# lyf8118/BDS-3-B1C-B2a-SDR-receiver

Hardware: AMD Instinct MI355X
Metric: IF Msamples/s through acquisition (all PRNs x Doppler bins) (higher is better)
Workload: dtype f32

## Files before the change

bds-3-b1c-b2a-sdr-receiver_amd/csrc/bds_acq.hip:

```cpp
#include <hip/hip_runtime.h>

#include <algorithm>
#include <array>
#include <cmath>
#include <cstdarg>
#include <cstdlib>
#include <map>
#include <set>
#include <tuple>

#include "bds_acq_scols.h"
#include "bds_acq_wcols.h"
#include "bds_acq_refine.h"
#include "bds_acq_wrows.h"
#include "bds_acq_pfa.h"
#include "bds_internal.h"

namespace bds {

static const double kPi = 3.14159265358979323846;

#include "bds_acq_plan.h"

struct EventPool {
// ... 1074 lines not shown
        dim3 gr(pl.L1, nb), gc(pl.ntiles, nb);
        if (ncomp == 2) {
            hipLaunchKernelGGL(k_rows_inv<2>, gr, dim3(pl.nt_rows), pl.lds_rows, s_main, pl.p2, pl.twl,
                               (const float2 *)a.d_Xs, pl.L, b0, Cs, a.d_Bw);
            hipLaunchKernelGGL(k_cols_inv_max<2>, gc, dim3(pl.nt_cols), pl.lds_cols, s_main, pl.p1, pl.L2, pl.logT,
                               pl.Spad, (const float2 *)a.d_Bw, pl.L, w0, w1, lo1, hi1, lo2, hi2, recs, pl.ntiles);
        } else {
            hipLaunchKernelGGL(k_rows_inv<1>, gr, dim3(pl.nt_rows), pl.lds_rows, s_main, pl.p2, pl.twl,
                               (const float2 *)a.d_Xs, pl.L, b0, Cs, a.d_Bw);
            hipLaunchKernelGGL(k_cols_inv_max<1>, gc, dim3(pl.nt_cols), pl.lds_cols, s_main, pl.p1, pl.L2, pl.logT,
                               pl.Spad, (const float2 *)a.d_Bw, pl.L, w0, w1, lo1, hi1, lo2, hi2, recs, pl.ntiles);
        }
    }
}

void AcqRun::launch_list(int ncells, Rec *recs, const CellList &cl, int cell0, hipEvent_t mid) {
    Plan2D &pl = a.plan;
    const hipStream_t s_main = stream();
    SieveOut so1 = so;
    so1.recs = recs;
    so1.cell0 = cell0;
    so1.mid = mid;
    if (mid) mids = true;
    const int hi1 = cl.rng ? -1 : (int)a.N - 1, lo2 = cl.rng ? 0 : 1, hi2 = cl.rng ? -1 : 0;
    if (pfa) {
        const int gc = std::max(1, cl.gc), chunks = (ncells + gc - 1) / gc;
        const size_t rows_lds = 2 * 3136 * sizeof(float2);
        want_lds(ctx, pfa::k_pfa_cols<2, false>, pfa::kColsLds);
        pfa::RowsArgs ra{(const uint32_t *)a.d_Xs, (const uint32_t *)a.d_Cs, (uint32_t *)a.d_Bw, cl.bin, cl.cs, ncells, gc, pfa};
        hipLaunchKernelGGL(pfa::k_pfa_rows<2>, dim3((unsigned)(pfa::MP * pfa::K2 * chunks)), dim3(pfa::kRowsThreads), rows_lds, s_main, ra);
        if (mid) (void)hipEventRecord(mid, s_main);
        const int qch = ctx->tune.pfa_qchunk > 0 ? ctx->tune.pfa_qchunk : 1;
        const long items = (long)((pfa::kTiles + qch - 1) / qch) * qch * ncells;
        const unsigned cgrid = (unsigned)std::min<long>(items, ctx->tune.pfa_cgrid > 0 ? ctx->tune.pfa_cgrid : std::max<long>(512, std::min<long>(8192, items / 24)));
        pfa::ColsArgs ca{(const uint32_t *)a.d_Bw, a.d_pfa_coef, ncells, w0, w1, so1.cellmax, so1.lb, so1.lb_div, so1.extra, so1.extra_count,
                         so1.extra_cap, cell0, so1.keep, qch, nullptr, nullptr, -1, -1};
        hipLaunchKernelGGL((pfa::k_pfa_cols<2, false>), dim3(cgrid), dim3(pfa::kColsThreads), pfa::kColsLds, s_main, ca);
        return;
    }
    if (a.half) {
        if (ncomp == 2)
            launch_fast_f<2, __half2>(ctx, s_main, pl, a.d_Xs, ncells, 0, a.d_Cs, a.d_Bw, a.sB, w0, w1, 0, hi1, lo2, hi2, so1, cl);
        else
            launch_fast_f<1, __half2>(ctx, s_main, pl, a.d_Xs, ncells, 0, a.d_Cs, a.d_Bw, a.sB, w0, w1, 0, hi1, lo2, hi2, so1, cl);
    } else {
        if (ncomp == 2)
            launch_fast_f<2, float2>(ctx, s_main, pl, a.d_Xs, ncells, 0, a.d_Cs, a.d_Bw, a.sB, w0, w1, 0, hi1, lo2, hi2, so1, cl);
        else
            launch_fast_f<1, float2>(ctx, s_main, pl, a.d_Xs, ncells, 0, a.d_Cs, a.d_Bw, a.sB, w0, w1, 0, hi1, lo2, hi2, so1, cl);
    }
}

int AcqRun::search() {
    Plan2D &pl = a.plan;
    const hipStream_t s_main = stream();
    int rc;
    const long sample_every = std::max<long>(1, n_pairs_total / kSamples);
    long pair_idx = 0, group_idx = 0;
    if (!multiprn && (rc = ensure_fit(ctx, &a.d_Bw, &a.bw_cap, bw_batches(a, ctx->tune) * (size_t)pl.L))) return rc;
    if (multiprn) {
        for (;;) {
            const size_t need = ((size_t)PB * D * cell_elems * elem + 7) / 8;
            if (!(rc = ensure_fit(ctx, &a.d_Bw, &a.bw_cap, std::max(need, bw_batches(a, ctx->tune) * (size_t)pl.L)))) break;
            if (PB <= 2) return rc;
            (void)hipGetLastError();
            PB = (PB + 1) / 2;
            a.pb_last = PB;
// ... 370 lines not shown
```

bds-3-b1c-b2a-sdr-receiver_amd/csrc/bds_acq_pfa.h:

```cpp
#pragma once

#include <hip/hip_fp16.h>
#include <hip/hip_runtime.h>

#include <type_traits>

#include "bds_acq_wcols.h"

namespace bds {
namespace pfa {

constexpr int K1 = 53, K2 = 12, K3 = 3125;
constexpr long NP = (long)K1 * K2 * K3;
constexpr int MP = 27;
constexpr int NB = 7;
constexpr int kTileLags = 16, kTiles = (K3 + kTileLags - 1) / kTileLags;
constexpr size_t kCellElems = (size_t)kTiles * MP * K2 * kTileLags * 4;
__host__ __device__ constexpr size_t bw_piece(int mp, int k2, int t3) {
    return (((size_t)(t3 / kTileLags) * MP + mp) * K2 + k2) * (kTileLags * 4) + (size_t)(t3 % kTileLags) * 4;
}
constexpr int kRowsThreads = 256, kColsThreads = 256;
constexpr int kCoefFrags = NB * 4 * 2;
constexpr size_t kCoefBytes = (size_t)kCoefFrags * 64 * 16;
constexpr size_t kColsLds = kCoefBytes + (size_t)NB * kColsThreads * 4;

typedef _Float16 h8 __attribute__((ext_vector_type(8)));
typedef float f4 __attribute__((ext_vector_type(4)));

__host__ __device__ inline long lag_of(int t1, int t2, int t3) {
    return ((long)t1 * (NP / K1) + (long)t2 * (NP / K2) + (long)t3 * (NP / K3)) % NP;
}

__device__ __forceinline__ void pk_radix5(v2f &x0, v2f &x1, v2f &x2, v2f &x3, v2f &x4) {
    constexpr float c1 = 0.30901699437494745f, c2 = -0.80901699437494734f, s1 = 0.95105651629515353f, s2 = 0.58778525229247314f;
    const v2f t1 = x1 + x4, t2 = x2 + x3, t3 = x1 - x4, t4 = x2 - x3;
    const v2f m1 = x0 + c1 * t1 + c2 * t2;
    const v2f m2 = x0 + c2 * t1 + c1 * t2;
    const v2f n1 = s1 * t3 + s2 * t4;
    const v2f n2 = s2 * t3 - s1 * t4;
    x0 = x0 + t1 + t2;
    x1 = pk_addj(m1, n1);
    x4 = pk_subj(m1, n1);
    x2 = pk_addj(m2, n2);
    x3 = pk_subj(m2, n2);
}

__device__ __forceinline__ v2f w25(int k) {
    constexpr float c[17] = {1.f, 0.9685831611286311f, 0.8763066800438636f, 0.7289686274214116f, 0.5358267949789965f, 0.30901699437494745f,
                             0.06279051952931353f, -0.1873813145857246f, -0.4257792915650727f, -0.6374239897486897f, -0.8090169943749473f,
                             -0.9297764858882513f, -0.9921147013144778f, -0.9921147013144779f, -0.9297764858882515f, -0.8090169943749478f,
                             -0.6374239897486895f};
    constexpr float s[17] = {0.f, 0.2486898871648548f, 0.4817536741017153f, 0.6845471059286886f, 0.8443279255020151f, 0.9510565162951535f,
                             0.9980267284282716f, 0.9822872507286887f, 0.9048270524660195f, 0.7705132427757893f, 0.5877852522924732f,
                             0.36812455268467814f, 0.12533323356430454f, -0.12533323356430429f, -0.3681245526846779f, -0.5877852522924727f,
                             -0.7705132427757894f};
    return (v2f){c[k], s[k]};
}

__device__ __forceinline__ void pk_radix25(v2f (&x)[25]) {
#pragma unroll
    for (int q0 = 0; q0 < 5; ++q0) pk_radix5(x[q0], x[q0 + 5], x[q0 + 10], x[q0 + 15], x[q0 + 20]);
#pragma unroll
    for (int q0 = 1; q0 < 5; ++q0)
#pragma unroll
// ... 141 lines not shown
#pragma unroll
            for (int sl = 0; sl < 25; ++sl) {
                const int tq = slot25_index(sl);
                typedef _Float16 h2 __attribute__((ext_vector_type(2)));
                outp[c][tq] = __builtin_bit_cast(uint32_t, __builtin_convertvector(x[sl], h2));
            }
        }
        asm volatile("" : "+v"(bin_next));
        bin_cur = __builtin_amdgcn_readfirstlane(bin_next);
        typedef int v4i __attribute__((ext_vector_type(4)));
        const unsigned long long dst_base = (unsigned long long)(A.Bw + (size_t)cell * kCellElems + bw_piece(mp, k2, 0));
        const v4i dst_words = {(int)(unsigned)dst_base, (int)((unsigned)(dst_base >> 32) & 0xffffu), (int)(unsigned)((kCellElems - bw_piece(mp, k2, 0)) * 4), 0x00020000};
#pragma unroll
        for (int e = 0; e < 25; e += 2) {
            uint32_t P[2], Q[2];
#pragma unroll
            for (int c = 0; c < 2; ++c) {
                const uint32_t pe = c < NC ? outp[c < NC ? c : 0][e] : 0u, qo = (c < NC && e + 1 < 25) ? outp[c < NC ? c : 0][e + 1 < 25 ? e + 1 : e] : 0u;
                const auto r = __builtin_amdgcn_permlane32_swap(pe, qo, false, false);
                P[c] = r[0], Q[c] = r[1];
            }
            const int tq = e + half;
            if (live && tq < 25) {
                typedef uint32_t u4 __attribute__((ext_vector_type(4)));
                const int t3s = j + 125 * tq;
                asm volatile("buffer_store_dwordx4 %0, %1, %2, 0 offen\n s_nop 0" ::"v"((u4){P[0], Q[0], P[1], Q[1]}), "v"((int)(bw_piece(0, 0, t3s) * 4)), "s"(dst_words)
                             : "memory");
            }
        }
        __syncthreads();
    }
}

inline void make_coef_frags(uint16_t *out ) {
    auto f2h = [](float f) { return __half_as_ushort(__float2half_rn(f)); };
    auto h2f = [](uint16_t h) { return __half2float(__ushort_as_half(h)); };
    for (int nb = 0; nb < NB; ++nb)
        for (int ins = 0; ins < 4; ++ins)
            for (int lane = 0; lane < 64; ++lane)
                for (int e = 0; e < 8; ++e) {
                    const int kap = 32 * ins + 8 * (lane >> 4) + e, o = 16 * nb + (lane & 15);
                    const int k1 = kap >> 1, ri = kap & 1, t1 = o >> 1, ro = o & 1;
                    double v = 0.0;
                    if (k1 < K1 && t1 < K1) {
                        const double ang = 2.0 * M_PI * (double)((k1 * t1) % K1) / K1;
                        const double c = cos(ang), s = sin(ang);
                        v = ro == 0 ? (ri == 0 ? c : -s) : (ri == 0 ? s : c);
                    }
                    const uint16_t hi = f2h((float)v);
                    const uint16_t lo = f2h((float)(v - (double)h2f(hi)));
                    out[((((size_t)nb * 4 + ins) * 2 + 0) * 64 + lane) * 8 + e] = hi;
                    out[((((size_t)nb * 4 + ins) * 2 + 1) * 64 + lane) * 8 + e] = lo;
                }
}

struct ColsArgs {
    const uint32_t *Bw;
    const uint4 *coef;
    int ncells;
    float w0, w1;
    unsigned long long *cellmax;
    float *lb;
    int lb_div;
    Extra *extra;
    int *extra_count;
    int extra_cap;
    int cell0;
    float keep;
    int qchunk;
    unsigned long long *stats;
    float *dbg;
    int dbg_cell, dbg_group;
};

__device__ __forceinline__ void real_dft6(float a0, float a1, float a2, float a3, float a4, float a5, float (&re)[4], float (&im)[4]) {
    constexpr float h3 = 0.86602540378443865f;
    const float s0 = a0 + a3, d0 = a0 - a3, s1 = a1 + a4, d1 = a1 - a4, s2 = a2 + a5, d2 = a2 - a5;
    const float s12 = s1 + s2, d12 = d1 - d2;
    re[0] = s0 + s12, im[0] = 0.f;
    re[2] = fmaf(-0.5f, s12, s0), im[2] = h3 * (s1 - s2);
    re[1] = fmaf(0.5f, d12, d0), im[1] = h3 * (d1 + d2);
    re[3] = d0 - d12, im[3] = 0.f;
}
__device__ __forceinline__ void real_dft12(const float (&v)[12], float (&P)[7], float (&Q)[7]) {
    float er[4], ei[4], orr[4], oi[4];
    real_dft6(v[0], v[2], v[4], v[6], v[8], v[10], er, ei);
    real_dft6(v[1], v[3], v[5], v[7], v[9], v[11], orr, oi);
    constexpr float c1 = 0.86602540378443865f, s1 = 0.5f;
    P[0] = er[0] + orr[0], Q[0] = 0.f;
    P[6] = er[0] - orr[0], Q[6] = 0.f;
    P[3] = er[3], Q[3] = orr[3];
    P[1] = er[1] + c1 * orr[1] - s1 * oi[1], Q[1] = ei[1] + c1 * oi[1] + s1 * orr[1];
    P[5] = er[1] - c1 * orr[1] + s1 * oi[1], Q[5] = -ei[1] + c1 * oi[1] + s1 * orr[1];
    P[2] = er[2] + s1 * orr[2] - c1 * oi[2], Q[2] = ei[2] + s1 * oi[2] + c1 * orr[2];
    P[4] = er[2] - s1 * orr[2] + c1 * oi[2], Q[4] = -ei[2] + s1 * oi[2] + c1 * orr[2];
}

template <int NC, bool DBG>
__global__ __launch_bounds__(kColsThreads, 2) void k_pfa_cols(ColsArgs A) {
    extern __shared__ __align__(16) unsigned char pfa_lds[];
    uint4 *s_coef = reinterpret_cast<uint4 *>(pfa_lds);
    float *s_bm = reinterpret_cast<float *>(pfa_lds + kCoefBytes);
    const int tid = threadIdx.x, wave = tid >> 6, lane = tid & 63;
    for (int i = tid; i < kCoefFrags * 64; i += kColsThreads) s_coef[i] = A.coef[i];
    __syncthreads();
    const int ai = lane & 15, g = ai >> 2, r = ai & 3, ks = lane >> 4;
    const bool odd = lane & 1;
    auto t2_of = [&](int i) { return odd ? (i == 0 ? 6 : 12 - i) : i; };
    constexpr int kBlocks = kTiles;
    const int qch = A.qchunk > 0 ? A.qchunk : 1, nq = (kBlocks + qch - 1) / qch;
    const unsigned ncl = (unsigned)A.ncells, uq = (unsigned)qch;
    unsigned b = blockIdx.x % uq, cl = (blockIdx.x / uq) % ncl, q = blockIdx.x / (uq * ncl);
    const unsigned gb = gridDim.x % uq, gcl = (gridDim.x / uq) % ncl, gq = gridDim.x / (uq * ncl);
    for (; q < (unsigned)nq; b += gb, cl += gcl + (b >= uq ? (b -= uq, 1u) : 0u), q += gq + (cl >= ncl ? (cl -= ncl, 1u) : 0u)) {
        const int blk = (int)(q * uq + b);
        const int t0 = 16 * blk + 4 * wave;
        if (blk >= kBlocks || t0 >= K3) continue;
        const int cell = A.cell0 + cl;
        float *const lbp = A.lb + cell / A.lb_div;
        const int t3 = min(t0 + g, K3 - 1);
        const uint32_t *base = A.Bw + (size_t)cl * kCellElems;
        uint4 fa[2][3][4];
#pragma unroll
        for (int quad = 0; quad < 3; ++quad)
#pragma unroll
            for (int ins = 0; ins < 4; ++ins) {
                const int mg = 4 * ins + ks;
                const size_t off = bw_piece(0, 4 * quad + r, t3);
                const uint4 l0 = *reinterpret_cast<const uint4 *>(base + (size_t)min(2 * mg, MP - 1) * K2 * (kTileLags * 4) + off);
                const uint4 l1 = *reinterpret_cast<const uint4 *>(base + (size_t)min(2 * mg + 1, MP - 1) * K2 * (kTileLags * 4) + off);
                fa[0][quad][ins] = make_uint4(l0.x, l0.y, l1.x, l1.y);
                fa[1][quad][ins] = make_uint4(l0.z, l0.w, l1.z, l1.w);
            }
        auto matrix = [&](int nb, f4 (&acc2)[NC][3], auto parts_tag) {
            constexpr int PARTS = decltype(parts_tag)::value;
            uint4 fb[4][2];
#pragma unroll
            for (int ins = 0; ins < 4; ++ins)
#pragma unroll
                for (int part = 0; part < PARTS; ++part) fb[ins][part] = s_coef[((nb * 4 + ins) * 2 + part) * 64 + lane];
#pragma unroll
            for (int c = 0; c < NC; ++c) {
#pragma unroll
                for (int quad = 0; quad < 3; ++quad) acc2[c][quad] = (f4){0.f, 0.f, 0.f, 0.f};
#pragma unroll
                for (int ins = 0; ins < 4; ++ins)
#pragma unroll
                    for (int part = 0; part < PARTS; ++part)
#pragma unroll
                        for (int quad = 0; quad < 3; ++quad)
                            acc2[c][quad] = __builtin_amdgcn_mfma_f32_16x16x32_f16(__builtin_bit_cast(h8, fa[c][quad][ins]), __builtin_bit_cast(h8, fb[ins][part]),
                                                                                   acc2[c][quad], 0, 0, 0);
            }
        };
        auto epilogue = [&](const f4 (&acc2)[NC][3], float (&m2)[2][6]) {
#pragma unroll
            for (int c = 0; c < NC; ++c) {
                const f4(&acc)[3] = acc2[c];
                float v[12], P[7], Q[7];
#pragma unroll
                for (int k = 0; k < 12; ++k) v[k] = acc[k >> 2][k & 3];
                real_dft12(v, P, Q);
                auto partner = [](float a) { return __builtin_bit_cast(float, __builtin_amdgcn_mov_dpp(__builtin_bit_cast(int, a), 0xB1, 0xf, 0xf, true)); };
                {
                    const float p0 = P[0] * P[0], p6 = P[6] * P[6];
                    const float S0 = p0 + partner(p0), S6 = p6 + partner(p6);
                    m2[c][0] = odd ? S6 : S0;
                }
#pragma unroll
                for (int t = 1; t < 6; ++t) {
                    const float sl = fmaf(Q[t], Q[t], P[t] * P[t]);
                    const float S = sl + partner(sl);
                    float x = partner(P[t]) * Q[t];
                    x = fmaf(-partner(Q[t]), P[t], x);
                    m2[c][t] = fmaf(2.f, x, S);
                }
            }
        };
        auto block = [&](int nb, float (&m2)[2][6], auto parts_tag) {
            f4 acc2[NC][3];
            matrix(nb, acc2, parts_tag);
            epilogue(acc2, m2);
        };
        const int t3o = t0 + (lane >> 4);
        constexpr int kParts1 = DBG ? 2 : 1;
        float best = 0.f, ssum = 0.f;
        f4 accp[2][NC][3];
        matrix(0, accp[0], std::integral_constant<int, kParts1>{});
        const float lbv = __hip_atomic_load(lbp, __ATOMIC_RELAXED, __HIP_MEMORY_SCOPE_AGENT);
        const unsigned cur = __hip_atomic_load(reinterpret_cast<const unsigned *>(A.cellmax + cell) + 1, __ATOMIC_RELAXED, __HIP_MEMORY_SCOPE_AGENT);
#pragma unroll
        for (int nb = 0; nb < NB; ++nb) {
            float m2[2][6];
            if (nb + 1 < NB) matrix(nb + 1, accp[(nb + 1) & 1], std::integral_constant<int, kParts1>{});
            epilogue(accp[nb & 1], m2);
            const int t1 = (16 * nb + (lane & 15)) >> 1;
            float bmax = 0.f, bsum = 0.f;
#pragma unroll
            for (int i = 0; i < 6; ++i) {
                const float e = NC == 2 ? m2[0][i] + m2[1][i] : m2[0][i];
                bmax = fmaxf(bmax, e), bsum += e;
            }
            if (!(t1 < K1 && t3o < K3)) bmax = 0.f, bsum = 0.f;
            best = fmaxf(best, bmax), ssum += bsum;
            s_bm[nb * kColsThreads + tid] = bmax;
            if (DBG && cell == A.dbg_cell && t0 / 4 == A.dbg_group && t1 < K1) {
#pragma unroll
                for (int c = 0; c < NC; ++c)
#pragma unroll
                    for (int i = 0; i < 6; ++i) A.dbg[((c * K1 + t1) * 12 + t2_of(i)) * 4 + (lane >> 4)] = m2[c][i];
            }
        }
        if (A.stats && lane == 0) atomicAdd(A.stats, 1ull);
        const float wsum2 = NC > 1 ? A.w0 * A.w0 + A.w1 * A.w1 : A.w0 * A.w0;
        float dlt = 0.f;
        if (kParts1 == 1) {
            float s16 = ssum;
            s16 += __builtin_bit_cast(float, __builtin_amdgcn_mov_dpp(__builtin_bit_cast(int, s16), 0x128, 0xf, 0xf, true));
            s16 += __builtin_bit_cast(float, __builtin_amdgcn_mov_dpp(__builtin_bit_cast(int, s16), 0x124, 0xf, 0xf, true));
            s16 += __builtin_bit_cast(float, __builtin_amdgcn_mov_dpp(__builtin_bit_cast(int, s16), 0x122, 0xf, 0xf, true));
            s16 += __builtin_bit_cast(float, __builtin_amdgcn_mov_dpp(__builtin_bit_cast(int, s16), 0x121, 0xf, 0xf, true));
            dlt = 5.0e-4f * sqrtf(s16);
        }
        const float ub = wave_max_f32(sqrtf(best) + dlt);
        const float bw = ub * ub * wsum2 * 1.00001f;
        const float curv = __uint_as_float(cur), lim = fminf(curv, lbv * A.keep);
        if (!(bw < lim * lim)) {
            if (A.stats && lane == 0) atomicAdd(A.stats + 1, 1ull);
            unsigned fmask = 0;
            for (int nb = 0; nb < NB; ++nb) {
                const float u = sqrtf(s_bm[nb * kColsThreads + tid]) + dlt;
                if (__builtin_amdgcn_ballot_w64(!(u * u * wsum2 * 1.00001f < lim * lim))) fmask |= 1u << nb;
            }
            if (A.stats && lane == 0) atomicAdd(A.stats + 3, (unsigned long long)__builtin_popcount(fmask));
            float top1 = -1.f, top2 = -1.f;
            int lag1 = 0x7fffffff, lag2 = 0x7fffffff;
            for (int nb = 0; nb < NB; ++nb) {
                if (!((fmask >> nb) & 1)) continue;
                float m2[2][6];
                block(nb, m2, std::integral_constant<int, 2>{});
                const int t1 = (16 * nb + (lane & 15)) >> 1;
                if (t1 < K1 && t3o < K3) {
#pragma unroll
                    for (int i = 0; i < 6; ++i) {
                        float a = A.w0 * __builtin_amdgcn_sqrtf(fmaxf(m2[0][i], 0.f));
                        if (NC > 1) a += A.w1 * __builtin_amdgcn_sqrtf(fmaxf(m2[NC - 1][i], 0.f));
                        const int lag = (int)lag_of(t1, t2_of(i), t3o);
                        if (a > top1 || (a == top1 && lag < lag1)) {
                            top2 = top1, lag2 = lag1, top1 = a, lag1 = lag;
                        } else if (a > top2 || (a == top2 && lag < lag2)) {
                            top2 = a, lag2 = lag;
                        }
                    }
                }
            }
            const float Mw = wave_max_f32(top1);
            if (Mw >= 0.f) {
                const float thr = fmaxf(Mw, lbv) * A.keep;
                const bool newmax = __float_as_uint(Mw) >= cur;
                const unsigned long long hit1 = __builtin_amdgcn_ballot_w64(top1 >= thr), hit2 = __builtin_amdgcn_ballot_w64(top2 >= thr);
                if (newmax || hit1) {
                    if (!hit2) {
                        const int total = __builtin_popcountll(hit1);
                        if (total > 0) {
                            int base_i = 0;
                            if (lane == 0) base_i = atomicAdd(A.extra_count, total);
                            base_i = __builtin_amdgcn_readfirstlane(base_i);
                            if (top1 >= thr) {
                                const int idx = base_i + (int)__builtin_amdgcn_mbcnt_hi((unsigned)(hit1 >> 32), __builtin_amdgcn_mbcnt_lo((unsigned)hit1, 0u));
                                if ((unsigned)idx < (unsigned)A.extra_cap) {
                                    Extra ex;
                                    ex.v = top1, ex.lag = lag1, ex.cell = cell;
                                    A.extra[idx] = ex;
                                }
                            }
                        }
                    } else {
                        if (A.stats && lane == 0) atomicAdd(A.stats + 2, 1ull);
                        for (int nb = 0; nb < NB; ++nb) {
                            if (!((fmask >> nb) & 1)) continue;
                            float m2[2][6];
                            block(nb, m2, std::integral_constant<int, 2>{});
                            const int t1 = (16 * nb + (lane & 15)) >> 1;
                            const bool mine = t1 < K1 && t3o < K3;
#pragma unroll
                            for (int i = 0; i < 6; ++i) {
                                float a = -1.f;
                                if (mine) {
                                    a = A.w0 * __builtin_amdgcn_sqrtf(fmaxf(m2[0][i], 0.f));
                                    if (NC > 1) a += A.w1 * __builtin_amdgcn_sqrtf(fmaxf(m2[NC - 1][i], 0.f));
                                }
                                const unsigned long long mask = __builtin_amdgcn_ballot_w64(a >= thr);
                                if (mask) {
                                    int base_i = 0;
                                    if (lane == 0) base_i = atomicAdd(A.extra_count, __builtin_popcountll(mask));
                                    base_i = __builtin_amdgcn_readfirstlane(base_i);
                                    if (a >= thr) {
                                        const int idx = base_i + (int)__builtin_amdgcn_mbcnt_hi((unsigned)(mask >> 32), __builtin_amdgcn_mbcnt_lo((unsigned)mask, 0u));
                                        if ((unsigned)idx < (unsigned)A.extra_cap) {
                                            Extra ex;
                                            ex.v = a, ex.lag = (int)lag_of(t1, t2_of(i), t3o), ex.cell = cell;
                                            A.extra[idx] = ex;
                                        }
                                    }
                                }
                            }
                        }
                    }
                    if (newmax) {
                        int bestlag = top1 == Mw ? lag1 : 0x7fffffff;
#pragma unroll
                        for (int o = 32; o > 0; o >>= 1) bestlag = min(bestlag, __shfl_xor(bestlag, o));
                        if (lane == 0) {
                            atomicMax(A.cellmax + cell, wc_pack(Mw, bestlag));
                            if (Mw > lbv) atomicMax(reinterpret_cast<unsigned *>(lbp), __float_as_uint(Mw));
                        }
                    }
                }
            }
        }
    }
}

template <class Loader>
__global__ __launch_bounds__(128) void k_pfa_fwd_rows(Loader ld, float2 *T ) {
    __shared__ float2 region[K3 + 11];
    const int row = blockIdx.x, batch = blockIdx.y, j = threadIdx.x;
    const bool live = j < 125;
    const int jj = live ? j : 124;
    const long base = ((long)(row / K2) * (NP / K1) + (long)(row % K2) * (NP / K2)) % NP;
    v2f x[25];
#pragma unroll
    for (int q = 0; q < 25; ++q) {
        const float2 v = ld(batch, (base + (long)(jj + 125 * q) * (NP / K3)) % NP);
        x[q] = (v2f){v.x, -v.y};
    }
    pk_radix25(x);
    if (live) {
#pragma unroll
        for (int sl = 0; sl < 25; ++sl) {
            const int p = slot25_index(sl);
            region[25 * j + p] = to_f2(p ? pk_cmul(x[sl], unit((jj * p) % K3, K3)) : x[sl]);
        }
    }
    __syncthreads();
    const int si = jj % 25, spg = jj / 25;
    if (live) {
#pragma unroll
        for (int c5 = 0; c5 < 5; ++c5) {
            v2f z[5];
#pragma unroll
            for (int r = 0; r < 5; ++r) z[r] = to_v2f(region[25 * (si + 25 * r) + 5 * spg + c5]);
            pk_radix5(z[0], z[1], z[2], z[3], z[4]);
#pragma unroll
// ... 89 lines not shown
```

Before: 183,300.

## Stage PFA column tiles into LDS with async loads shared by two wave teams

The columns kernel grows to 512 threads split into two 4-wave teams that share one LDS tile slot. Each tile is fetched with global_load_lds straight into LDS, using an XOR swizzle, and the next team's tile request is issued mid-computation behind barrier handshakes, so global latency overlaps with MFMA work. Coefficient and bound-matrix LDS accesses move to inline-asm ds_read/ds_write with compile-time offsets, and the host grid is halved to match. This adds a larger LDS footprint, barrier coupling between the teams, and fragile hand-written waitcnt sequencing.

```diff
diff --git a/bds-3-b1c-b2a-sdr-receiver_amd/csrc/bds_acq.hip b/bds-3-b1c-b2a-sdr-receiver_amd/csrc/bds_acq.hip
--- a/bds-3-b1c-b2a-sdr-receiver_amd/csrc/bds_acq.hip
+++ b/bds-3-b1c-b2a-sdr-receiver_amd/csrc/bds_acq.hip
@@ -1130,7 +1130,7 @@
         if (mid) (void)hipEventRecord(mid, s_main);
         const int qch = ctx->tune.pfa_qchunk > 0 ? ctx->tune.pfa_qchunk : 1;
         const long items = (long)((pfa::kTiles + qch - 1) / qch) * qch * ncells;
-        const unsigned cgrid = (unsigned)std::min<long>(items, ctx->tune.pfa_cgrid > 0 ? ctx->tune.pfa_cgrid : std::max<long>(512, std::min<long>(8192, items / 24)));
+        const unsigned cgrid = (unsigned)std::min<long>((items + 1) / 2, ctx->tune.pfa_cgrid > 0 ? ctx->tune.pfa_cgrid : std::max<long>(256, std::min<long>(4096, items / 48)));
         pfa::ColsArgs ca{(const uint32_t *)a.d_Bw, a.d_pfa_coef, ncells, w0, w1, so1.cellmax, so1.lb, so1.lb_div, so1.extra, so1.extra_count,
                          so1.extra_cap, cell0, so1.keep, qch, nullptr, nullptr, -1, -1};
         hipLaunchKernelGGL((pfa::k_pfa_cols<2, false>), dim3(cgrid), dim3(pfa::kColsThreads), pfa::kColsLds, s_main, ca);
diff --git a/bds-3-b1c-b2a-sdr-receiver_amd/csrc/bds_acq_pfa.h b/bds-3-b1c-b2a-sdr-receiver_amd/csrc/bds_acq_pfa.h
--- a/bds-3-b1c-b2a-sdr-receiver_amd/csrc/bds_acq_pfa.h
+++ b/bds-3-b1c-b2a-sdr-receiver_amd/csrc/bds_acq_pfa.h
@@ -19,10 +19,14 @@
 __host__ __device__ constexpr size_t bw_piece(int mp, int k2, int t3) {
     return (((size_t)(t3 / kTileLags) * MP + mp) * K2 + k2) * (kTileLags * 4) + (size_t)(t3 % kTileLags) * 4;
 }
-constexpr int kRowsThreads = 256, kColsThreads = 256;
+constexpr int kRowsThreads = 256, kColsThreads = 512;
 constexpr int kCoefFrags = NB * 4 * 2;
 constexpr size_t kCoefBytes = (size_t)kCoefFrags * 64 * 16;
-constexpr size_t kColsLds = kCoefBytes + (size_t)NB * kColsThreads * 4;
+constexpr size_t kTileBytes = (size_t)MP * K2 * kTileLags * 16;
+constexpr int kTileChunks = (int)(kTileBytes / 1024);
+static_assert(kTileBytes % 1024 == 0, "a tile is a whole number of 1 KiB wave-loads");
+constexpr size_t kColsBmOff = kCoefBytes, kColsSlotOff = kColsBmOff + (size_t)NB * kColsThreads * 4;
+constexpr size_t kColsLds = kColsSlotOff + kTileBytes;
 
 typedef _Float16 h8 __attribute__((ext_vector_type(8)));
 typedef float f4 __attribute__((ext_vector_type(4)));
@@ -301,49 +305,122 @@
     P[4] = er[2] - s1 * orr[2] + c1 * oi[2], Q[4] = -ei[2] + s1 * oi[2] + c1 * orr[2];
 }
 
+typedef uint32_t u4 __attribute__((ext_vector_type(4)));
+template <int PARTS, int OFF>
+__device__ __forceinline__ void lds_read_coef(u4 (&fb)[4][2], unsigned a) {
+    if constexpr (PARTS == 1) {
+        asm volatile("ds_read_b128 %0, %4 offset:%5\n ds_read_b128 %1, %4 offset:%5+2048\n ds_read_b128 %2, %4 offset:%5+4096\n ds_read_b128 %3, %4 offset:%5+6144\n s_waitcnt lgkmcnt(0)"
+                     : "=&v"(fb[0][0]), "=&v"(fb[1][0]), "=&v"(fb[2][0]), "=&v"(fb[3][0])
+                     : "v"(a), "n"(OFF)
+                     : "memory");
+    } else {
+        asm volatile(
+            "ds_read_b128 %0, %8 offset:%9\n ds_read_b128 %1, %8 offset:%9+1024\n ds_read_b128 %2, %8 offset:%9+2048\n ds_read_b128 %3, %8 offset:%9+3072\n"
+            "ds_read_b128 %4, %8 offset:%9+4096\n ds_read_b128 %5, %8 offset:%9+5120\n ds_read_b128 %6, %8 offset:%9+6144\n ds_read_b128 %7, %8 offset:%9+7168\n s_waitcnt lgkmcnt(0)"
+            : "=&v"(fb[0][0]), "=&v"(fb[0][1]), "=&v"(fb[1][0]), "=&v"(fb[1][1]), "=&v"(fb[2][0]), "=&v"(fb[2][1]), "=&v"(fb[3][0]), "=&v"(fb[3][1])
+            : "v"(a), "n"(OFF)
+            : "memory");
+    }
+}
+
 template <int NC, bool DBG>
 __global__ __launch_bounds__(kColsThreads, 2) void k_pfa_cols(ColsArgs A) {
     extern __shared__ __align__(16) unsigned char pfa_lds[];
     uint4 *s_coef = reinterpret_cast<uint4 *>(pfa_lds);
-    float *s_bm = reinterpret_cast<float *>(pfa_lds + kCoefBytes);
-    const int tid = threadIdx.x, wave = tid >> 6, lane = tid & 63;
+    const int tid = threadIdx.x, lane = tid & 63;
+    const int wave = __builtin_amdgcn_readfirstlane(tid >> 6), team = wave >> 2, tw = wave & 3;
     for (int i = tid; i < kCoefFrags * 64; i += kColsThreads) s_coef[i] = A.coef[i];
-    __syncthreads();
-    const int ai = lane & 15, g = ai >> 2, r = ai & 3, ks = lane >> 4;
+    const unsigned coef_a = lds_offset(pfa_lds) + (unsigned)lane * 16u;
+    const unsigned bm_a = lds_offset(pfa_lds) + (unsigned)kColsBmOff + (unsigned)tid * 4u;
+    unsigned char *const s_tile = pfa_lds + kColsSlotOff;
+    const int g = (lane & 15) >> 2;
     const bool odd = lane & 1;
     auto t2_of = [&](int i) { return odd ? (i == 0 ? 6 : 12 - i) : i; };
     constexpr int kBlocks = kTiles;
     const int qch = A.qchunk > 0 ? A.qchunk : 1, nq = (kBlocks + qch - 1) / qch;
     const unsigned ncl = (unsigned)A.ncells, uq = (unsigned)qch;
-    unsigned b = blockIdx.x % uq, cl = (blockIdx.x / uq) % ncl, q = blockIdx.x / (uq * ncl);
-    const unsigned gb = gridDim.x % uq, gcl = (gridDim.x / uq) % ncl, gq = gridDim.x / (uq * ncl);
-    for (; q < (unsigned)nq; b += gb, cl += gcl + (b >= uq ? (b -= uq, 1u) : 0u), q += gq + (cl >= ncl ? (cl -= ncl, 1u) : 0u)) {
+    const unsigned n_items = (unsigned)nq * uq * ncl;
+    const unsigned wg_items = blockIdx.x < n_items ? (n_items - blockIdx.x + gridDim.x - 1) / gridDim.x : 0u;
+    const unsigned trips = (wg_items + 1) / 2;
+    const unsigned first = blockIdx.x + (unsigned)team * gridDim.x, step = 2 * gridDim.x;
+    unsigned b = first % uq, cl = (first / uq) % ncl, q = first / (uq * ncl);
+    const unsigned gb = step % uq, gcl = (step / uq) % ncl, gq = step / (uq * ncl);
+    auto request_tile = [&](unsigned tb, unsigned tcl, unsigned tq) {
+        if (tq >= (unsigned)nq || tq * uq + tb >= (unsigned)kBlocks) return;
+        unsigned ln = (unsigned)lane;
+        asm volatile("" : "+v"(ln));
+        const unsigned char *src = reinterpret_cast<const unsigned char *>(A.Bw + (size_t)tcl * kCellElems) + (size_t)(tq * uq + tb) * kTileBytes +
+                                   (size_t)(tw * 1024) + (size_t)((ln ^ (((ln >> 4) & 3u) << 2)) * 16u);
+        unsigned char *dst = s_tile + tw * 1024;
+#pragma unroll
+        for (int k = 0; k < (kTileChunks + 3) / 4; ++k)
+            if (4 * k + tw < kTileChunks)
+                __builtin_amdgcn_global_load_lds((const __attribute__((address_space(1))) void *)(src + (size_t)k * 4096),
+                                                 (__attribute__((address_space(3))) void *)(dst + (size_t)k * 4096), 16, 0, 0);
+    };
+    auto slot_ready = [] {
+        __builtin_amdgcn_s_waitcnt(0x0070);
+        __builtin_amdgcn_s_barrier();
+        asm volatile("" ::: "memory");
+    };
+    auto slot_free = [] {
+        asm volatile("" ::: "memory");
+        __builtin_amdgcn_s_waitcnt(0xc07f);
+        __builtin_amdgcn_s_barrier();
+    };
+    if (team == 0) {
+        request_tile(b, cl, q);
+    } else {
+        slot_ready();
+        slot_free();
+        request_tile(b, cl, q);
+    }
+    for (unsigned trip = 0; trip < trips; ++trip) {
         const int blk = (int)(q * uq + b);
-        const int t0 = 16 * blk + 4 * wave;
-        if (blk >= kBlocks || t0 >= K3) continue;
+        const int t0 = 16 * blk + 4 * tw;
+        const bool work = q < (unsigned)nq && blk < kBlocks && t0 < K3;
+        if (!work) {
+            slot_ready();
+            slot_free();
+            b += gb, cl += gcl + (b >= uq ? (b -= uq, 1u) : 0u), q += gq + (cl >= ncl ? (cl -= ncl, 1u) : 0u);
+            slot_ready();
+            slot_free();
+            request_tile(b, cl, q);
+            continue;
+        }
         const int cell = A.cell0 + cl;
         float *const lbp = A.lb + cell / A.lb_div;
         const int t3 = min(t0 + g, K3 - 1);
-        const uint32_t *base = A.Bw + (size_t)cl * kCellElems;
         uint4 fa[2][3][4];
-#pragma unroll
-        for (int quad = 0; quad < 3; ++quad)
-#pragma unroll
-            for (int ins = 0; ins < 4; ++ins) {
-                const int mg = 4 * ins + ks;
-                const size_t off = bw_piece(0, 4 * quad + r, t3);
-                const uint4 l0 = *reinterpret_cast<const uint4 *>(base + (size_t)min(2 * mg, MP - 1) * K2 * (kTileLags * 4) + off);
-                const uint4 l1 = *reinterpret_cast<const uint4 *>(base + (size_t)min(2 * mg + 1, MP - 1) * K2 * (kTileLags * 4) + off);
-                fa[0][quad][ins] = make_uint4(l0.x, l0.y, l1.x, l1.y);
-                fa[1][quad][ins] = make_uint4(l0.z, l0.w, l1.z, l1.w);
-            }
-        auto matrix = [&](int nb, f4 (&acc2)[NC][3], auto parts_tag) {
+        slot_ready();
+        {
+            constexpr int kPairBytes = K2 * kTileLags * 16, kQuadBytes = 4 * kTileLags * 16;
+            int ln = lane;
+            asm volatile("" : "+v"(ln));
+            const int fr = ln & 3, fks = ln >> 4;
+            const unsigned char *piece = s_tile + fr * 256 + (((t3 - 16 * blk) ^ (fr << 2)) << 4);
+            const unsigned char *p0 = piece + 2 * fks * kPairBytes;
+            const unsigned char *pa = piece + min(24 + 2 * fks, MP - 1) * kPairBytes, *pb = piece + min(25 + 2 * fks, MP - 1) * kPairBytes;
+#pragma unroll
+            for (int quad = 0; quad < 3; ++quad)
+#pragma unroll
+                for (int ins = 0; ins < 4; ++ins) {
+                    const uint4 l0 = *reinterpret_cast<const uint4 *>(ins < 3 ? p0 + 8 * ins * kPairBytes + quad * kQuadBytes : pa + quad * kQuadBytes);
+                    const uint4 l1 = *reinterpret_cast<const uint4 *>(ins < 3 ? p0 + (8 * ins + 1) * kPairBytes + quad * kQuadBytes : pb + quad * kQuadBytes);
+                    fa[0][quad][ins] = make_uint4(l0.x, l0.y, l1.x, l1.y);
+                    fa[1][quad][ins] = make_uint4(l0.z, l0.w, l1.z, l1.w);
+                }
+        }
+        slot_free();
+        b += gb, cl += gcl + (b >= uq ? (b -= uq, 1u) : 0u), q += gq + (cl >= ncl ? (cl -= ncl, 1u) : 0u);
+        auto matrix = [&](auto nb, f4 (&acc2)[NC][3], auto parts_tag) {
             constexpr int PARTS = decltype(parts_tag)::value;
-            uint4 fb[4][2];
-#pragma unroll
-            for (int ins = 0; ins < 4; ++ins)
-#pragma unroll
-                for (int part = 0; part < PARTS; ++part) fb[ins][part] = s_coef[((nb * 4 + ins) * 2 + part) * 64 + lane];
+            u4 fb[4][2];
+            constexpr int kBlockBytes = 4 * 2 * 64 * 16;
+            if constexpr (std::is_same_v<decltype(nb), int>)
+                lds_read_coef<PARTS, 0>(fb, coef_a + (unsigned)nb * kBlockBytes);
+            else
+                lds_read_coef<PARTS, decltype(nb)::value * kBlockBytes>(fb, coef_a);
 #pragma unroll
             for (int c = 0; c < NC; ++c) {
 #pragma unroll
@@ -389,15 +466,15 @@
         };
         const int t3o = t0 + (lane >> 4);
         constexpr int kParts1 = DBG ? 2 : 1;
+        constexpr int kSplit = 3;
         float best = 0.f, ssum = 0.f;
         f4 accp[2][NC][3];
-        matrix(0, accp[0], std::integral_constant<int, kParts1>{});
-        const float lbv = __hip_atomic_load(lbp, __ATOMIC_RELAXED, __HIP_MEMORY_SCOPE_AGENT);
-        const unsigned cur = __hip_atomic_load(reinterpret_cast<const unsigned *>(A.cellmax + cell) + 1, __ATOMIC_RELAXED, __HIP_MEMORY_SCOPE_AGENT);
-#pragma unroll
-        for (int nb = 0; nb < NB; ++nb) {
+        float lbv = 0.f;
+        unsigned cur = 0u;
+        auto bound_block = [&](auto nb_tag) {
+            constexpr int nb = decltype(nb_tag)::value;
             float m2[2][6];
-            if (nb + 1 < NB) matrix(nb + 1, accp[(nb + 1) & 1], std::integral_constant<int, kParts1>{});
+            if constexpr (nb + 1 < NB) matrix(std::integral_constant<int, nb + 1>{}, accp[(nb + 1) & 1], std::integral_constant<int, kParts1>{});
             epilogue(accp[nb & 1], m2);
             const int t1 = (16 * nb + (lane & 15)) >> 1;
             float bmax = 0.f, bsum = 0.f;
@@ -408,14 +485,24 @@
             }
             if (!(t1 < K1 && t3o < K3)) bmax = 0.f, bsum = 0.f;
             best = fmaxf(best, bmax), ssum += bsum;
-            s_bm[nb * kColsThreads + tid] = bmax;
+            asm volatile("ds_write_b32 %0, %1 offset:%2" ::"v"(bm_a), "v"(bmax), "n"(nb * kColsThreads * 4) : "memory");
             if (DBG && cell == A.dbg_cell && t0 / 4 == A.dbg_group && t1 < K1) {
 #pragma unroll
                 for (int c = 0; c < NC; ++c)
 #pragma unroll
                     for (int i = 0; i < 6; ++i) A.dbg[((c * K1 + t1) * 12 + t2_of(i)) * 4 + (lane >> 4)] = m2[c][i];
             }
-        }
+        };
+        {
+            matrix(std::integral_constant<int, 0>{}, accp[0], std::integral_constant<int, kParts1>{});
+            lbv = __hip_atomic_load(lbp, __ATOMIC_RELAXED, __HIP_MEMORY_SCOPE_AGENT);
+            cur = __hip_atomic_load(reinterpret_cast<const unsigned *>(A.cellmax + cell) + 1, __ATOMIC_RELAXED, __HIP_MEMORY_SCOPE_AGENT);
+            static_for<kSplit>([&](auto i) { bound_block(i); });
+        }
+        slot_ready();
+        slot_free();
+        request_tile(b, cl, q);
+        static_for<NB - kSplit>([&](auto i) { bound_block(std::integral_constant<int, kSplit + decltype(i)::value>{}); });
         if (A.stats && lane == 0) atomicAdd(A.stats, 1ull);
         const float wsum2 = NC > 1 ? A.w0 * A.w0 + A.w1 * A.w1 : A.w0 * A.w0;
         float dlt = 0.f;
@@ -434,7 +521,9 @@
             if (A.stats && lane == 0) atomicAdd(A.stats + 1, 1ull);
             unsigned fmask = 0;
             for (int nb = 0; nb < NB; ++nb) {
-                const float u = sqrtf(s_bm[nb * kColsThreads + tid]) + dlt;
+                float bmv;
+                asm volatile("ds_read_b32 %0, %1\n s_waitcnt lgkmcnt(0)" : "=v"(bmv) : "v"(bm_a + (unsigned)nb * (kColsThreads * 4)) : "memory");
+                const float u = sqrtf(bmv) + dlt;
                 if (__builtin_amdgcn_ballot_w64(!(u * u * wsum2 * 1.00001f < lim * lim))) fmask |= 1u << nb;
             }
             if (A.stats && lane == 0) atomicAdd(A.stats + 3, (unsigned long long)__builtin_popcount(fmask));
@@ -525,6 +614,10 @@
             }
         }
     }
+    if (team == 0) {
+        slot_ready();
+        slot_free();
+    }
 }
 
 template <class Loader>
```

Result: slower. 179,900 (-1.9%).

## Exploit real-input symmetry in the K1 DFT to halve MFMA work

Applied to the files above, without the earlier changes.

Restructures the column-stage 53-point DFT so the coefficient matrix uses only the cos/sin of real inputs with Hermitian symmetry. This cuts the column blocks from 7 to 4 and the MFMA k-steps from 4 to 2 per block, and each lane now produces all 12 t2 outputs by combining the real and imaginary channel DFTs through a DPP partner exchange. Loads switch to buffer loads with byte permutes, and lag computation is simplified with an incremental lag_at. The risk is correctness of the symmetric reconstruction and extra epilogue ALU work per block.

```diff
diff --git a/bds-3-b1c-b2a-sdr-receiver_amd/csrc/bds_acq_pfa.h b/bds-3-b1c-b2a-sdr-receiver_amd/csrc/bds_acq_pfa.h
--- a/bds-3-b1c-b2a-sdr-receiver_amd/csrc/bds_acq_pfa.h
+++ b/bds-3-b1c-b2a-sdr-receiver_amd/csrc/bds_acq_pfa.h
@@ -13,23 +13,32 @@
 constexpr int K1 = 53, K2 = 12, K3 = 3125;
 constexpr long NP = (long)K1 * K2 * K3;
 constexpr int MP = 27;
-constexpr int NB = 7;
+constexpr int NB = 4;
 constexpr int kTileLags = 16, kTiles = (K3 + kTileLags - 1) / kTileLags;
 constexpr size_t kCellElems = (size_t)kTiles * MP * K2 * kTileLags * 4;
 __host__ __device__ constexpr size_t bw_piece(int mp, int k2, int t3) {
     return (((size_t)(t3 / kTileLags) * MP + mp) * K2 + k2) * (kTileLags * 4) + (size_t)(t3 % kTileLags) * 4;
 }
 constexpr int kRowsThreads = 256, kColsThreads = 256;
-constexpr int kCoefFrags = NB * 4 * 2;
+constexpr int kCoefFrags = NB * 2 * 2;
 constexpr size_t kCoefBytes = (size_t)kCoefFrags * 64 * 16;
 constexpr size_t kColsLds = kCoefBytes + (size_t)NB * kColsThreads * 4;
 
 typedef _Float16 h8 __attribute__((ext_vector_type(8)));
 typedef float f4 __attribute__((ext_vector_type(4)));
 
-__host__ __device__ inline long lag_of(int t1, int t2, int t3) {
+__host__ __device__ constexpr long lag_of(int t1, int t2, int t3) {
     return ((long)t1 * (NP / K1) + (long)t2 * (NP / K2) + (long)t3 * (NP / K3)) % NP;
 }
+__host__ __device__ constexpr int lag_base(int t1, int t3) { return (int)(((unsigned)t1 * (unsigned)(NP / K1) + (unsigned)t3 * (unsigned)(NP / K3)) % (unsigned)NP); }
+__host__ __device__ constexpr int lag_at(int lb0, int t2) { return lb0 + t2 * (int)(NP / K2) >= (int)NP ? lb0 + t2 * (int)(NP / K2) - (int)NP : lb0 + t2 * (int)(NP / K2); }
+constexpr bool lag_maps_agree(int t3) {
+    for (int t1 = 0; t1 < K1; ++t1)
+        for (int t2 = 0; t2 < K2; ++t2)
+            if (lag_at(lag_base(t1, t3), t2) != lag_of(t1, t2, t3)) return false;
+    return true;
+}
+static_assert(lag_maps_agree(0) && lag_maps_agree(1) && lag_maps_agree(1562) && lag_maps_agree(K3 - 2) && lag_maps_agree(K3 - 1), "lag_at / lag_base against lag_of");
 
 __device__ __forceinline__ void pk_radix5(v2f &x0, v2f &x1, v2f &x2, v2f &x3, v2f &x4) {
     constexpr float c1 = 0.30901699437494745f, c2 = -0.80901699437494734f, s1 = 0.95105651629515353f, s2 = 0.58778525229247314f;
@@ -237,25 +246,25 @@
     }
 }
 
+__host__ __device__ constexpr int coef_row(int ins, int ks, int e) { return 32 * ins + 8 * (e >> 1) + 2 * ks + (e & 1); }
 inline void make_coef_frags(uint16_t *out ) {
     auto f2h = [](float f) { return __half_as_ushort(__float2half_rn(f)); };
     auto h2f = [](uint16_t h) { return __half2float(__ushort_as_half(h)); };
     for (int nb = 0; nb < NB; ++nb)
-        for (int ins = 0; ins < 4; ++ins)
+        for (int ins = 0; ins < 2; ++ins)
             for (int lane = 0; lane < 64; ++lane)
                 for (int e = 0; e < 8; ++e) {
-                    const int kap = 32 * ins + 8 * (lane >> 4) + e, o = 16 * nb + (lane & 15);
-                    const int k1 = kap >> 1, ri = kap & 1, t1 = o >> 1, ro = o & 1;
+                    const int k1 = coef_row(ins, lane >> 4, e), o = 16 * nb + (lane & 15);
+                    const int t = o >> 1;
                     double v = 0.0;
-                    if (k1 < K1 && t1 < K1) {
-                        const double ang = 2.0 * M_PI * (double)((k1 * t1) % K1) / K1;
-                        const double c = cos(ang), s = sin(ang);
-                        v = ro == 0 ? (ri == 0 ? c : -s) : (ri == 0 ? s : c);
+                    if (k1 < K1 && o < 2 * MP && o != 1) {
+                        const double ang = 2.0 * M_PI * (double)((k1 * t) % K1) / K1;
+                        v = (o & 1) ? sin(ang) : cos(ang);
                     }
                     const uint16_t hi = f2h((float)v);
                     const uint16_t lo = f2h((float)(v - (double)h2f(hi)));
-                    out[((((size_t)nb * 4 + ins) * 2 + 0) * 64 + lane) * 8 + e] = hi;
-                    out[((((size_t)nb * 4 + ins) * 2 + 1) * 64 + lane) * 8 + e] = lo;
+                    out[((((size_t)nb * 2 + ins) * 2 + 0) * 64 + lane) * 8 + e] = hi;
+                    out[((((size_t)nb * 2 + ins) * 2 + 1) * 64 + lane) * 8 + e] = lo;
                 }
 }
 
@@ -311,7 +320,7 @@
     __syncthreads();
     const int ai = lane & 15, g = ai >> 2, r = ai & 3, ks = lane >> 4;
     const bool odd = lane & 1;
-    auto t2_of = [&](int i) { return odd ? (i == 0 ? 6 : 12 - i) : i; };
+    const int lane_piece = (int)(bw_piece(ks, r, 0) * 4);
     constexpr int kBlocks = kTiles;
     const int qch = A.qchunk > 0 ? A.qchunk : 1, nq = (kBlocks + qch - 1) / qch;
     const unsigned ncl = (unsigned)A.ncells, uq = (unsigned)qch;
@@ -323,98 +332,136 @@
         if (blk >= kBlocks || t0 >= K3) continue;
         const int cell = A.cell0 + cl;
         float *const lbp = A.lb + cell / A.lb_div;
-        const int t3 = min(t0 + g, K3 - 1);
-        const uint32_t *base = A.Bw + (size_t)cl * kCellElems;
-        uint4 fa[2][3][4];
-#pragma unroll
-        for (int quad = 0; quad < 3; ++quad)
-#pragma unroll
-            for (int ins = 0; ins < 4; ++ins) {
-                const int mg = 4 * ins + ks;
-                const size_t off = bw_piece(0, 4 * quad + r, t3);
-                const uint4 l0 = *reinterpret_cast<const uint4 *>(base + (size_t)min(2 * mg, MP - 1) * K2 * (kTileLags * 4) + off);
-                const uint4 l1 = *reinterpret_cast<const uint4 *>(base + (size_t)min(2 * mg + 1, MP - 1) * K2 * (kTileLags * 4) + off);
-                fa[0][quad][ins] = make_uint4(l0.x, l0.y, l1.x, l1.y);
-                fa[1][quad][ins] = make_uint4(l0.z, l0.w, l1.z, l1.w);
-            }
-        auto matrix = [&](int nb, f4 (&acc2)[NC][3], auto parts_tag) {
+        const int lag_in = min(4 * wave + g, K3 - 1 - 16 * blk);
+        const __amdgpu_buffer_rsrc_t bw_rsrc =
+            __builtin_amdgcn_make_buffer_rsrc((void *)(A.Bw + (size_t)cl * kCellElems + bw_piece(0, 0, 16 * blk)), 0, (int)(bw_piece(MP, 0, 0) * 4), 0x00020000);
+        const int voff = lane_piece + lag_in * 16;
+        const int voff6 = voff - (ks == 3 ? K2 * kTileLags * 16 : 0);
+        uint4 fa[2][2][3][2];
+#pragma unroll
+        for (int quad = 0; quad < 3; ++quad) {
+            uint32_t w[2][2][8];
+#pragma unroll
+            for (int p = 0; p < 8; ++p) {
+                if (4 * p >= MP) {
+                    w[0][0][p] = w[0][1][p] = w[1][0][p] = w[1][1][p] = 0u;
+                    continue;
+                }
+                typedef unsigned u4 __attribute__((ext_vector_type(4)));
+                const u4 l = __builtin_bit_cast(u4, __builtin_amdgcn_raw_buffer_load_b128(bw_rsrc, 4 * p + 3 < MP ? voff : voff6,
+                                                                                          (int)(bw_piece(4 * p, 4 * quad, 0) * 4), 0));
+                w[0][0][p] = __builtin_amdgcn_perm(l.y, l.x, 0x05040100u), w[0][1][p] = __builtin_amdgcn_perm(l.y, l.x, 0x07060302u);
+                w[1][0][p] = __builtin_amdgcn_perm(l.w, l.z, 0x05040100u), w[1][1][p] = __builtin_amdgcn_perm(l.w, l.z, 0x07060302u);
+            }
+#pragma unroll
+            for (int c = 0; c < 2; ++c)
+#pragma unroll
+                for (int ri = 0; ri < 2; ++ri)
+#pragma unroll
+                    for (int ins = 0; ins < 2; ++ins)
+                        fa[c][ri][quad][ins] = make_uint4(w[c][ri][4 * ins], w[c][ri][4 * ins + 1], w[c][ri][4 * ins + 2], w[c][ri][4 * ins + 3]);
+        }
+        auto coefs = [&](int nb, uint4 (&fb)[2][2], auto parts_tag) {
             constexpr int PARTS = decltype(parts_tag)::value;
-            uint4 fb[4][2];
-#pragma unroll
-            for (int ins = 0; ins < 4; ++ins)
-#pragma unroll
-                for (int part = 0; part < PARTS; ++part) fb[ins][part] = s_coef[((nb * 4 + ins) * 2 + part) * 64 + lane];
+#pragma unroll
+            for (int ins = 0; ins < 2; ++ins)
+#pragma unroll
+                for (int part = 0; part < PARTS; ++part) fb[ins][part] = s_coef[((nb * 2 + ins) * 2 + part) * 64 + lane];
+        };
+        auto matrix = [&](int c, const uint4 (&fb)[2][2], f4 (&acc)[2][3], auto parts_tag) {
+            constexpr int PARTS = decltype(parts_tag)::value;
+#pragma unroll
+            for (int ri = 0; ri < 2; ++ri)
+#pragma unroll
+                for (int quad = 0; quad < 3; ++quad) acc[ri][quad] = (f4){0.f, 0.f, 0.f, 0.f};
+#pragma unroll
+            for (int ins = 0; ins < 2; ++ins)
+#pragma unroll
+                for (int part = 0; part < PARTS; ++part)
+#pragma unroll
+                    for (int ri = 0; ri < 2; ++ri)
+#pragma unroll
+                        for (int quad = 0; quad < 3; ++quad)
+                            acc[ri][quad] = __builtin_amdgcn_mfma_f32_16x16x32_f16(__builtin_bit_cast(h8, fa[c][ri][quad][ins]), __builtin_bit_cast(h8, fb[ins][part]),
+                                                                                   acc[ri][quad], 0, 0, 0);
+        };
+        auto epilogue = [&](const f4 (&acc)[2][3], float (&m)[12]) {
+            float va[12], vb[12], Pa[7], Qa[7], Pb[7], Qb[7];
+#pragma unroll
+            for (int k = 0; k < 12; ++k) va[k] = acc[0][k >> 2][k & 3], vb[k] = acc[1][k >> 2][k & 3];
+            real_dft12(va, Pa, Qa);
+            __builtin_amdgcn_sched_barrier(0x18c);
+            real_dft12(vb, Pb, Qb);
+            __builtin_amdgcn_sched_barrier(0x18c);
+            auto partner = [](float a) { return __builtin_bit_cast(float, __builtin_amdgcn_mov_dpp(__builtin_bit_cast(int, a), 0xB1, 0xf, 0xf, true)); };
+            auto out = [&](float wr, float wi) {
+                const float yr = wr - partner(wi), yi = wi + partner(wr);
+                return fmaf(yi, yi, yr * yr);
+            };
+            m[0] = out(Pa[0], Pb[0]);
+            m[6] = out(Pa[6], Pb[6]);
+#pragma unroll
+            for (int t = 1; t < 6; ++t) {
+                m[t] = out(Pa[t] - Qb[t], Qa[t] + Pb[t]);
+                m[12 - t] = out(Pa[t] + Qb[t], Pb[t] - Qa[t]);
+            }
+        };
+        auto block = [&](int nb, float (&m2)[2][12], auto parts_tag) {
+            uint4 fb[2][2];
+            coefs(nb, fb, parts_tag);
 #pragma unroll
             for (int c = 0; c < NC; ++c) {
-#pragma unroll
-                for (int quad = 0; quad < 3; ++quad) acc2[c][quad] = (f4){0.f, 0.f, 0.f, 0.f};
-#pragma unroll
-                for (int ins = 0; ins < 4; ++ins)
-#pragma unroll
-                    for (int part = 0; part < PARTS; ++part)
-#pragma unroll
-                        for (int quad = 0; quad < 3; ++quad)
-                            acc2[c][quad] = __builtin_amdgcn_mfma_f32_16x16x32_f16(__builtin_bit_cast(h8, fa[c][quad][ins]), __builtin_bit_cast(h8, fb[ins][part]),
-                                                                                   acc2[c][quad], 0, 0, 0);
-            }
-        };
-        auto epilogue = [&](const f4 (&acc2)[NC][3], float (&m2)[2][6]) {
-#pragma unroll
-            for (int c = 0; c < NC; ++c) {
-                const f4(&acc)[3] = acc2[c];
-                float v[12], P[7], Q[7];
-#pragma unroll
-                for (int k = 0; k < 12; ++k) v[k] = acc[k >> 2][k & 3];
-                real_dft12(v, P, Q);
-                auto partner = [](float a) { return __builtin_bit_cast(float, __builtin_amdgcn_mov_dpp(__builtin_bit_cast(int, a), 0xB1, 0xf, 0xf, true)); };
-                {
-                    const float p0 = P[0] * P[0], p6 = P[6] * P[6];
-                    const float S0 = p0 + partner(p0), S6 = p6 + partner(p6);
-                    m2[c][0] = odd ? S6 : S0;
-                }
-#pragma unroll
-                for (int t = 1; t < 6; ++t) {
-                    const float sl = fmaf(Q[t], Q[t], P[t] * P[t]);
-                    const float S = sl + partner(sl);
-                    float x = partner(P[t]) * Q[t];
-                    x = fmaf(-partner(Q[t]), P[t], x);
-                    m2[c][t] = fmaf(2.f, x, S);
-                }
-            }
-        };
-        auto block = [&](int nb, float (&m2)[2][6], auto parts_tag) {
-            f4 acc2[NC][3];
-            matrix(nb, acc2, parts_tag);
-            epilogue(acc2, m2);
+                f4 acc[2][3];
+                matrix(c, fb, acc, parts_tag);
+                epilogue(acc, m2[c]);
+#pragma unroll
+                for (int i = 0; i < 12; ++i) asm volatile("" : "+v"(m2[c][i]));
+            }
         };
         const int t3o = t0 + (lane >> 4);
+        auto t1_of = [&](int nb) {
+            const int o = 16 * nb + (lane & 15), t = o >> 1, t1 = odd ? K1 - t : t;
+            return (o < 2 * MP && t1 < K1) ? t1 : -1;
+        };
         constexpr int kParts1 = DBG ? 2 : 1;
+        const std::integral_constant<int, kParts1> parts1{};
         float best = 0.f, ssum = 0.f;
-        f4 accp[2][NC][3];
-        matrix(0, accp[0], std::integral_constant<int, kParts1>{});
+        constexpr int NU = NB * NC;
+        f4 accp[2][2][3];
+        uint4 fbp[2][2];
+        coefs(0, fbp, parts1);
+        matrix(0, fbp, accp[0], parts1);
         const float lbv = __hip_atomic_load(lbp, __ATOMIC_RELAXED, __HIP_MEMORY_SCOPE_AGENT);
         const unsigned cur = __hip_atomic_load(reinterpret_cast<const unsigned *>(A.cellmax + cell) + 1, __ATOMIC_RELAXED, __HIP_MEMORY_SCOPE_AGENT);
-#pragma unroll
-        for (int nb = 0; nb < NB; ++nb) {
-            float m2[2][6];
-            if (nb + 1 < NB) matrix(nb + 1, accp[(nb + 1) & 1], std::integral_constant<int, kParts1>{});
-            epilogue(accp[nb & 1], m2);
-            const int t1 = (16 * nb + (lane & 15)) >> 1;
+        float mfirst[12];
+#pragma unroll
+        for (int u = 0; u < NU; ++u) {
+            const int nb = u / NC, c = u % NC;
+            float m[12];
+            if (u + 1 < NU) {
+                if ((u + 1) % NC == 0) coefs((u + 1) / NC, fbp, parts1);
+                matrix((u + 1) % NC, fbp, accp[(u + 1) & 1], parts1);
+            }
+            epilogue(accp[u & 1], m);
+            const int t1 = t1_of(nb);
+            if (DBG && cell == A.dbg_cell && t0 / 4 == A.dbg_group && t1 >= 0) {
+#pragma unroll
+                for (int i = 0; i < 12; ++i) A.dbg[((c * K1 + t1) * 12 + i) * 4 + (lane >> 4)] = m[i];
+            }
+            if (c + 1 < NC) {
+#pragma unroll
+                for (int i = 0; i < 12; ++i) mfirst[i] = m[i];
+                continue;
+            }
             float bmax = 0.f, bsum = 0.f;
 #pragma unroll
-            for (int i = 0; i < 6; ++i) {
-                const float e = NC == 2 ? m2[0][i] + m2[1][i] : m2[0][i];
+            for (int i = 0; i < 12; ++i) {
+                const float e = NC == 2 ? mfirst[i] + m[i] : m[i];
                 bmax = fmaxf(bmax, e), bsum += e;
             }
-            if (!(t1 < K1 && t3o < K3)) bmax = 0.f, bsum = 0.f;
+            if (!(t1 >= 0 && t3o < K3)) bmax = 0.f, bsum = 0.f;
             best = fmaxf(best, bmax), ssum += bsum;
             s_bm[nb * kColsThreads + tid] = bmax;
-            if (DBG && cell == A.dbg_cell && t0 / 4 == A.dbg_group && t1 < K1) {
-#pragma unroll
-                for (int c = 0; c < NC; ++c)
-#pragma unroll
-                    for (int i = 0; i < 6; ++i) A.dbg[((c * K1 + t1) * 12 + t2_of(i)) * 4 + (lane >> 4)] = m2[c][i];
-            }
         }
         if (A.stats && lane == 0) atomicAdd(A.stats, 1ull);
         const float wsum2 = NC > 1 ? A.w0 * A.w0 + A.w1 * A.w1 : A.w0 * A.w0;
@@ -442,15 +489,16 @@
             int lag1 = 0x7fffffff, lag2 = 0x7fffffff;
             for (int nb = 0; nb < NB; ++nb) {
                 if (!((fmask >> nb) & 1)) continue;
-                float m2[2][6];
+                float m2[2][12];
                 block(nb, m2, std::integral_constant<int, 2>{});
-                const int t1 = (16 * nb + (lane & 15)) >> 1;
-                if (t1 < K1 && t3o < K3) {
-#pragma unroll
-                    for (int i = 0; i < 6; ++i) {
+                const int t1 = t1_of(nb);
+                if (t1 >= 0 && t3o < K3) {
+                    const int lb0 = lag_base(t1, t3o);
+#pragma unroll
+                    for (int i = 0; i < 12; ++i) {
                         float a = A.w0 * __builtin_amdgcn_sqrtf(fmaxf(m2[0][i], 0.f));
                         if (NC > 1) a += A.w1 * __builtin_amdgcn_sqrtf(fmaxf(m2[NC - 1][i], 0.f));
-                        const int lag = (int)lag_of(t1, t2_of(i), t3o);
+                        const int lag = lag_at(lb0, i);
                         if (a > top1 || (a == top1 && lag < lag1)) {
                             top2 = top1, lag2 = lag1, top1 = a, lag1 = lag;
                         } else if (a > top2 || (a == top2 && lag < lag2)) {
@@ -484,12 +532,13 @@
                         if (A.stats && lane == 0) atomicAdd(A.stats + 2, 1ull);
                         for (int nb = 0; nb < NB; ++nb) {
                             if (!((fmask >> nb) & 1)) continue;
-                            float m2[2][6];
+                            float m2[2][12];
                             block(nb, m2, std::integral_constant<int, 2>{});
-                            const int t1 = (16 * nb + (lane & 15)) >> 1;
-                            const bool mine = t1 < K1 && t3o < K3;
-#pragma unroll
-                            for (int i = 0; i < 6; ++i) {
+                            const int t1 = t1_of(nb);
+                            const bool mine = t1 >= 0 && t3o < K3;
+                            const int lb0 = lag_base(mine ? t1 : 0, t3o);
+#pragma unroll
+                            for (int i = 0; i < 12; ++i) {
                                 float a = -1.f;
                                 if (mine) {
                                     a = A.w0 * __builtin_amdgcn_sqrtf(fmaxf(m2[0][i], 0.f));
@@ -504,7 +553,7 @@
                                         const int idx = base_i + (int)__builtin_amdgcn_mbcnt_hi((unsigned)(mask >> 32), __builtin_amdgcn_mbcnt_lo((unsigned)mask, 0u));
                                         if ((unsigned)idx < (unsigned)A.extra_cap) {
                                             Extra ex;
-                                            ex.v = a, ex.lag = (int)lag_of(t1, t2_of(i), t3o), ex.cell = cell;
+                                            ex.v = a, ex.lag = lag_at(lb0, i), ex.cell = cell;
                                             A.extra[idx] = ex;
                                         }
                                     }
```

After: 192,800 before, 197,300 after, median of 6. 2.3% higher.
